# jan-hofmeier/pathnet-gym

Hardware: AMD Instinct MI355X
Metric: env_frames_per_sec_whole_node_pong_pathnet (higher is better)
Workload: dtype fp32x

## Files before the change

csrc/trunk_x3.hip:

```cpp
#include "common.h"
#include <type_traits>

namespace x3 {

#define X3_NCX 3
#define X3_MAXM 16
#define X3_NCT 5
#define X3_RING_FCS 1024
#define X3_C1_FWD_FCS 128
#define X3_W0_SHIFT 8

template <int HIN_, int WIN_, int CIN_, int KH_, int KW_, int S_, bool U8_>
struct CG {
  static constexpr int HIN = HIN_, WIN = WIN_, CIN = CIN_, KH = KH_, KW = KW_, S = S_;
  static constexpr bool U8 = U8_;
  static constexpr int HO = (HIN - KH) / S + 1, WO = (WIN - KW) / S + 1, HOWO = HO * WO;
  static constexpr int K = KH * KW * CIN, KP = (K + 31) / 32 * 32, KC = KP / 8;
  static constexpr int IN_ELEMS = HIN * WIN * CIN;
};
using C1 = CG<160, 120, 4, 8, 8, 4, true>;
using C2 = CG<39, 29, 8, 4, 4, 2, false>;
using C3 = CG<18, 13, 8, 3, 3, 1, false>;

typedef __bf16 b2v __attribute__((ext_vector_type(2)));
// ... 2734 lines not shown

template <int COUT>
__global__ __launch_bounds__(256) void fc_gm_x3(const float* __restrict__ G, const uint16_t* __restrict__ bits,
                                                const int* __restrict__ act_cnt, int layer, int L, int P, int E, int T,
                                                long bits_rows, float g_scale, bf16_t* __restrict__ Gm, long gmlo,
                                                const float* __restrict__ gamax) {
  constexpr int NW = COUT / 16, C8 = COUT / 8;
  const int R = T * E;
  const long idx = (long)blockIdx.x * 256 + threadIdx.x;
  const long row = idx / C8;
  const int c = (int)(idx - row * C8) * 8;
  if (row >= (long)P * R) return;
  const int p = (int)(row / R), r = (int)(row - (long)p * R);
  const int cnt = act_cnt[p * L + layer];
  const long sg = sample_global(p, r, E, P * E, 0);
  const float4 a0 = *reinterpret_cast<const float4*>(G + sg * COUT + c);
  const float4 a1 = *reinterpret_cast<const float4*>(G + sg * COUT + c + 4);
  const float gv[8] = {a0.x * g_scale, a0.y * g_scale, a0.z * g_scale, a0.w * g_scale,
                       a1.x * g_scale, a1.y * g_scale, a1.z * g_scale, a1.w * g_scale};
  const float gs = g16_scale(gamax);
  for (int a = 0; a < cnt; ++a) {
    const uint32_t bw = (uint32_t)bits[((long)a * bits_rows + sg) * NW + (c >> 4)] >> (c & 15);
    float m[8];
#pragma unroll
    for (int j = 0; j < 8; ++j) m[j] = ((bw >> j) & 1u) ? gv[j] : 0.f;
    s8v hi, lo;
    split8hs(m, gs, hi, lo);
    bf16_t* gp = Gm + ((long)a * bits_rows + sg) * COUT + c;
    *reinterpret_cast<s8v*>(gp) = hi;
    *reinterpret_cast<s8v*>(gp + gmlo) = lo;
  }
}

template <int COUT, bool W3 = false, int FOLD = 0>
__global__ __launch_bounds__(512) void fc_dgrad_gemm_x3(const bf16_t* __restrict__ Gm, long gmlo,
                                                        const bf16_t* __restrict__ WcT, long wlo,
                                                        const int* __restrict__ act_idx,
                                                        const int* __restrict__ act_cnt, int layer, int L, int M, int K,
                                                        int KP, int P, int E, int T, long bits_rows,
                                                        float* __restrict__ dX, int nrb, int ncb,
                                                        const float* __restrict__ gamax, float* __restrict__ gamax_out) {
  constexpr int BM = 128, BN = 256, CS = COUT / 32;
  constexpr int NBP = W3 ? 3 : 2;
  __shared__ __attribute__((aligned(16))) bf16_t As[2][2][BM * 32];
  __shared__ __attribute__((aligned(16))) bf16_t Bs[2][NBP][BN * 32];
  const int ntot = P * nrb * ncb, per = (ntot + 7) >> 3, kx = (int)(blockIdx.x >> 3);
  const int bid = (int)(blockIdx.x & 7) * per + kx;
  if (kx >= per || bid >= ntot) return;
  const int p = bid / (nrb * ncb), rem = bid - p * (nrb * ncb);
  const int rbk = rem / ncb, cb = rem - rbk * ncb;
  const int R = T * E, PE = P * E;
  const int cnt = act_cnt[p * L + layer];
  const int tid = threadIdx.x, w = tid >> 6, l = tid & 63;
  const int grp = l >> 4, c16 = l & 15;
  const int wm = w >> 2, wn = w & 3;
  const int row0 = rbk * BM, col0 = cb * BN;
  const int nsteps = cnt * CS;
  f4v acc[4][4], accn[FOLD == 2 ? 4 : 1][FOLD == 2 ? 4 : 1];
#pragma unroll
  for (int i = 0; i < 4; ++i)
#pragma unroll
    for (int jj = 0; jj < 4; ++jj) acc[i][jj] = (f4v){0.f, 0.f, 0.f, 0.f};
  if constexpr (FOLD == 2) {
#pragma unroll
    for (int i = 0; i < 4; ++i)
#pragma unroll
      for (int jj = 0; jj < 4; ++jj) accn[i][jj] = (f4v){0.f, 0.f, 0.f, 0.f};
  }
  if (nsteps > 0) {
    const int sr = tid >> 2, sk = tid & 3;
    const int ra = min(row0 + sr, R - 1);
    const long asg = sample_global(p, ra, E, PE, 0);
    const int kb0 = min(col0 + sr, K - 1), kb1 = min(col0 + 128 + sr, K - 1);
    const int* aidx = act_idx + (p * L + layer) * M;
    const int sdA = mm2_sw(sr, sk) * 8, sdB0 = sdA, sdB1 = mm2_sw(sr + 128, sk) * 8;
    uint4 x0, x1, y0, y1, z0, z1, u0, u1, v0, v1, t0_, t1_, r0, r1, q0, q1;
#define DG_LOAD(S, st)                                                                                      \
    do {                                                                                                    \
      const int a_ = (st) / CS, c_ = ((st) - a_ * CS) * 32 + sk * 8;                                        \
      const bf16_t* ga_ = Gm + ((long)a_ * bits_rows + asg) * COUT + c_;                                    \
      const bf16_t* wb_ = WcT + (long)aidx[a_] * KP * COUT + c_;                                            \
      x##S = *reinterpret_cast<const uint4*>(ga_);                                                          \
      y##S = *reinterpret_cast<const uint4*>(ga_ + gmlo);                                                   \
      z##S = *reinterpret_cast<const uint4*>(wb_ + (long)kb0 * COUT);                                       \
      u##S = *reinterpret_cast<const uint4*>(wb_ + wlo + (long)kb0 * COUT);                                 \
      v##S = *reinterpret_cast<const uint4*>(wb_ + (long)kb1 * COUT);                                       \
      t##S##_ = *reinterpret_cast<const uint4*>(wb_ + wlo + (long)kb1 * COUT);                              \
      if constexpr (W3) {                                                                                   \
        r##S = *reinterpret_cast<const uint4*>(wb_ + 2 * wlo + (long)kb0 * COUT);                           \
        q##S = *reinterpret_cast<const uint4*>(wb_ + 2 * wlo + (long)kb1 * COUT);                           \
      }                                                                                                     \
    } while (0)
#define DG_STORE(S, buf)                                                                                    \
    do {                                                                                                    \
      if (FOLD == 2 && (buf) == 1) {              \
        x##S.x ^= 0x80008000u; x##S.y ^= 0x80008000u; x##S.z ^= 0x80008000u; x##S.w ^= 0x80008000u;         \
        y##S.x ^= 0x80008000u; y##S.y ^= 0x80008000u; y##S.z ^= 0x80008000u; y##S.w ^= 0x80008000u;         \
      }                                                                                                     \
      *reinterpret_cast<uint4*>(&As[buf][0][sdA]) = x##S;                                                   \
      *reinterpret_cast<uint4*>(&As[buf][1][sdA]) = y##S;                                                   \
      *reinterpret_cast<uint4*>(&Bs[buf][0][sdB0]) = z##S;                                                  \
      *reinterpret_cast<uint4*>(&Bs[buf][1][sdB0]) = u##S;                                                  \
      *reinterpret_cast<uint4*>(&Bs[buf][0][sdB1]) = v##S;                                                  \
      *reinterpret_cast<uint4*>(&Bs[buf][1][sdB1]) = t##S##_;                                               \
      if constexpr (W3) {                                                                                   \
        *reinterpret_cast<uint4*>(&Bs[buf][NBP - 1][sdB0]) = r##S;                                          \
        *reinterpret_cast<uint4*>(&Bs[buf][NBP - 1][sdB1]) = q##S;                                          \
      }                                                                                                     \
    } while (0)
    auto compute = [&](int buf) {
      s8v bh[4], bl[4], br[W3 ? 4 : 1];
#pragma unroll
      for (int jj = 0; jj < 4; ++jj) {
        const int o = mm2_sw(wn * 64 + jj * 16 + c16, grp) * 8;
        bh[jj] = *reinterpret_cast<const s8v*>(&Bs[buf][0][o]);
        bl[jj] = *reinterpret_cast<const s8v*>(&Bs[buf][1][o]);
        if constexpr (W3) br[jj] = *reinterpret_cast<const s8v*>(&Bs[buf][NBP - 1][o]);
      }
#pragma unroll
      for (int i = 0; i < 4; ++i) {
        const int o = mm2_sw(wm * 64 + i * 16 + c16, grp) * 8;
        const s8v ah = *reinterpret_cast<const s8v*>(&As[buf][0][o]);
        const s8v al = *reinterpret_cast<const s8v*>(&As[buf][1][o]);
#pragma unroll
        for (int jj = 0; jj < 4; ++jj) {
          if constexpr (FOLD == 2) {
            if (buf == 1) {
// ... 28 lines not shown
    if (s < nsteps) compute(0);
#undef DG_LOAD
#undef DG_STORE
  }
  const float inv = 1.0f / (g16_scale(gamax) * (float)(1 << X3_W0_SHIFT));
  float am = 0.f;
  if constexpr (FOLD == 2) {
#pragma unroll
    for (int i = 0; i < 4; ++i)
#pragma unroll
      for (int jj = 0; jj < 4; ++jj) acc[i][jj] -= accn[i][jj];
  }
#pragma unroll
  for (int i = 0; i < 4; ++i) {
#pragma unroll
    for (int r = 0; r < 4; ++r) {
      const int row = row0 + wm * 64 + i * 16 + 4 * grp + r;
      if (row >= R) continue;
      float* o = dX + sample_global(p, row, E, PE, 0) * (long)K;
#pragma unroll
      for (int jj = 0; jj < 4; ++jj) {
        const int k = col0 + wn * 64 + jj * 16 + c16;
        if (k < K) {
          const float v = acc[i][jj][r] * inv;
          o[k] = v;
          am = fmaxf(am, fabsf(v));
        }
      }
    }
  }
  g16_flush_amax(am, gamax_out);
}

template <int COUT, int KT = 128>
__global__ __launch_bounds__(512) void fc_wgrad_gm_x3(const bf16_t* __restrict__ X, long xlo, int ldx,
                                                      const bf16_t* __restrict__ Gm, long gmlo,
                                                      float* __restrict__ grad, long w_off, long b_off, int chunk,
                                                      const int* __restrict__ inv_path,
                                                      const int* __restrict__ inv_slot,
                                                      const int* __restrict__ inv_cnt, int layer, int M, int Pmax,
                                                      int K, int P, int E, int T, long bits_rows, int nsplit,
                                                      const float* __restrict__ gamax, long long* __restrict__ fx) {
  constexpr int XS = KT + 8;
  constexpr int MI = KT / 64;
  constexpr int XC = KT / 128;
  constexpr int GS = COUT + 8;
  constexpr int NT = COUT / 32;
  __shared__ __attribute__((aligned(16))) bf16_t Xs[2][2][32 * XS];
  __shared__ __attribute__((aligned(16))) bf16_t Gsh[2][2][32 * GS];
  const int kt = (K + KT - 1) / KT;
  const int zt = blockIdx.x / kt, tile_k = blockIdx.x - zt * kt;
  const int j = zt / nsplit, split = zt - j * nsplit;
  const int n_all = inv_cnt[layer * M + j];
  const int u_beg = (int)((long)n_all * split / nsplit), u_end = (int)((long)n_all * (split + 1) / nsplit);
  if (u_beg >= u_end) return;
  const int k0 = tile_k * KT;
  const int tid = threadIdx.x, w = tid >> 6, l = tid & 63;
  const int grp = l >> 4, i16 = l & 15, q = i16 >> 2, pp = i16 & 3;
  const int wk = w >> 1, wn = w & 1;
  const int Rtot = T * E, PE = P * E;
  const int nrb = (Rtot + 31) / 32;
  const int n_it = (u_end - u_beg) * nrb;
  const int* ip = inv_path + (layer * M + j) * Pmax;
  const int* is = inv_slot + (layer * M + j) * Pmax;
  constexpr int GSEG = COUT / 16;
  const int lr = tid >> 4, lxs = (tid & 15) * 8, lgs = (tid & 15) * GSEG;
  s8v xrh[XC], xrl[XC], grh[GSEG / 8], grl[GSEG / 8];
  auto gload = [&](int it) {
    const int ui = it / nrb;
    const int r = (it - ui * nrb) * 32 + lr;
    const int p = ip[u_beg + ui], a = is[u_beg + ui];
    const s8v z = (s8v){0, 0, 0, 0, 0, 0, 0, 0};
#pragma unroll
    for (int c = 0; c < XC; ++c) { xrh[c] = z; xrl[c] = z; }
#pragma unroll
    for (int h = 0; h < GSEG / 8; ++h) { grh[h] = z; grl[h] = z; }
    if (r < Rtot) {
      const long sg = sample_global(p, r, E, PE, 0);
#pragma unroll
      for (int c = 0; c < XC; ++c) {
        if (k0 + lxs + 128 * c < K) {
          xrh[c] = *reinterpret_cast<const s8v*>(X + sg * ldx + k0 + lxs + 128 * c);
          xrl[c] = *reinterpret_cast<const s8v*>(X + xlo + sg * ldx + k0 + lxs + 128 * c);
        }
      }
      const bf16_t* gp = Gm + ((long)a * bits_rows + sg) * COUT + lgs;
#pragma unroll
      for (int h = 0; h < GSEG / 8; ++h) {
        grh[h] = *reinterpret_cast<const s8v*>(gp + 8 * h);
        grl[h] = *reinterpret_cast<const s8v*>(gp + gmlo + 8 * h);
      }
    }
  };
  f4v acc[MI][NT];
#pragma unroll
  for (int i = 0; i < MI; ++i)
#pragma unroll
    for (int jj = 0; jj < NT; ++jj) acc[i][jj] = {0.f, 0.f, 0.f, 0.f};
  float bsum[NT];
#pragma unroll
  for (int jj = 0; jj < NT; ++jj) bsum[jj] = 0.f;
  const bool do_bias = tile_k == 0 && wk == 0;
  gload(0);
  for (int it = 0; it < n_it; ++it) {
    const int buf = it & 1;
#pragma unroll
    for (int c = 0; c < XC; ++c) {
      *reinterpret_cast<s8v*>(Xs[buf][0] + lr * XS + lxs + 128 * c) = xrh[c];
      *reinterpret_cast<s8v*>(Xs[buf][1] + lr * XS + lxs + 128 * c) = xrl[c];
    }
#pragma unroll
    for (int h = 0; h < GSEG / 8; ++h) {
      *reinterpret_cast<s8v*>(Gsh[buf][0] + lr * GS + lgs + 8 * h) = grh[h];
      *reinterpret_cast<s8v*>(Gsh[buf][1] + lr * GS + lgs + 8 * h) = grl[h];
    }
    __syncthreads();
    if (it + 1 < n_it) gload(it + 1);
    s8v afh[MI], afl[MI];
#pragma unroll
    for (int i = 0; i < MI; ++i) {
      const int o0 = (8 * grp + q) * XS + (KT / 4) * wk + 16 * i + 4 * pp;
      const int o1 = (8 * grp + 4 + q) * XS + (KT / 4) * wk + 16 * i + 4 * pp;
      afh[i] = tr8(Xs[buf][0] + o0, Xs[buf][0] + o1);
      afl[i] = tr8(Xs[buf][1] + o0, Xs[buf][1] + o1);
    }
#pragma unroll
    for (int jj = 0; jj < NT; ++jj) {
      const int nb = (COUT / 2) * wn + 16 * jj;
      const int o0 = (8 * grp + q) * GS + nb + 4 * pp, o1 = (8 * grp + 4 + q) * GS + nb + 4 * pp;
      const s8v bh = tr8(Gsh[buf][0] + o0, Gsh[buf][0] + o1);
      const s8v bl = tr8(Gsh[buf][1] + o0, Gsh[buf][1] + o1);
#pragma unroll
      for (int i = 0; i < MI; ++i) acc[i][jj] = mma3h(afh[i], afl[i], bh, bl, acc[i][jj]);
      if (do_bias) {
#pragma unroll
        for (int e = 0; e < 8; ++e) bsum[jj] += h2f((uint16_t)bh[e]) + h2f((uint16_t)bl[e]);
      }
    }
  }
  const long base = w_off + (long)j * chunk;
  const float ginv = 1.0f / g16_scale(gamax);
#pragma unroll
  for (int i = 0; i < MI; ++i)
#pragma unroll
    for (int jj = 0; jj < NT; ++jj)
// ... 244 lines not shown
  return Hin == G::HIN && Win == G::WIN && Cin == G::CIN && KH == G::KH && KW == G::KW && S == G::S &&
         (u8 != 0) == G::U8;
}

static int X3_WGRAD_PF = 3;
static int X3_C1_WG_NCX = 2;
static int X3_FC_KS = 1;
static int X3_FC_MMV = 3;
static int X3_FC_FWD_WPE = 0;
static int X3_C1_F16B = 1;
static int X3_C1_SB1 = 0;
static int X3_C1_EMAJ = 1;
static int X3_C1_BAL = 1;
static int X3_DG_W3 = 0;
static int X3_DG_FOLD = 2;
static int X3_WG_TARGET = 1536;
static int X3_WG_AUTO = 1;
static int X3_WG2_TARGET = 512;
static int X3_DG3_TARGET = 512;
static int X3_FC_RT1 = 2;
static int X3_C1F_TARGET = 512;
static int X3_C1F_MINB = 2;
static int X3_C23_TARGET = 512;
static int X3_C23_MINS = 1;
static int X3_WG3_TARGET = 256;
static int X3_FCW_TARGET = 1024;
static int X3_PRESPLIT = 1;
static int X3_DG_BAL = 1;
static int X3_DG_V0 = 0;
static int X3_DG_GSPLIT = X3_DG_SPLIT;
static int X3_DG_TARGET = 512;
static int X3_FC_KS_PARTS = 0;
static int X3_FC_DG_GEMM = 1;

template <auto KERN, int CAP>
static size_t lds_cap_pad() {
  static const size_t pad = [] {
    hipFuncAttributes a;
    if (hipFuncGetAttributes(&a, reinterpret_cast<const void*>(KERN)) != hipSuccess) return (size_t)0;
    const long need = 160L * 1024 / (CAP + 1) + 1;
    return need > (long)a.sharedSizeBytes ? (size_t)(need - (long)a.sharedSizeBytes) : (size_t)0;
  }();
  return pad;
}

long long* g_fx_accum = nullptr;

extern "C" {

int x3_set_fx(void* fx) {
  g_fx_accum = reinterpret_cast<long long*>(fx);
  return 0;
}

int x3_fx_flush(void* fx, float* grad, long n0, long n1, hipStream_t st) {
  if (!fx || !grad || n0 < 0 || n1 < n0) return -22;
  if (n1 == n0) return 0;
  long blocks = (n1 - n0 + 255) / 256;
  if (blocks > 2048) blocks = 2048;
  fx_flush_kernel<<<(unsigned)blocks, 256, 0, st>>>(reinterpret_cast<long long*>(fx), grad, n0, n1);
  return (int)hipGetLastError();
}

void fast_conv_set_x3_c1_wg_ncx(int v) { X3_C1_WG_NCX = v == 2 ? 2 : 3; }
void fast_conv_set_x3_fc_mmv(int v) { X3_FC_MMV = v; }
void fast_conv_set_x3_fc_fwd_wpe(int v) { X3_FC_FWD_WPE = v == 2 || v == 4 ? v : 0; }
void fast_conv_set_x3_fc_dg_gemm(int v) { X3_FC_DG_GEMM = v; }
void fast_conv_set_x3_dg_w3(int v) { X3_DG_W3 = v; }
void fast_conv_set_x3_dg_fold(int v) { X3_DG_FOLD = v; }
void fast_conv_set_x3_dg_v0(int v) { X3_DG_V0 = v; }
void fast_conv_set_x3_dg_bal(int v) { X3_DG_BAL = v; }
void fast_conv_set_x3_dg_gsplit(int v) { X3_DG_GSPLIT = v == 1 ? 1 : X3_DG_SPLIT; }
void fast_conv_set_x3_c1_bal(int v) { X3_C1_BAL = v; }
void fast_conv_set_x3_c1_emaj(int v) { X3_C1_EMAJ = v; }
void fast_conv_set_x3_c1_sb1(int v) { X3_C1_SB1 = v; }
void fast_conv_set_x3_c1_f16b(int v) { X3_C1_F16B = v; }
void fast_conv_set_x3_fc_ks(int ks) { X3_FC_KS = ks; }
void fast_conv_set_x3_wgrad_pf(int pf) { X3_WGRAD_PF = pf; }
void fast_conv_set_x3_presplit(int v) { X3_PRESPLIT = v ? 1 : 0; }
void fast_conv_set_x3_fc_rt1(int v) { X3_FC_RT1 = v; }
void fast_conv_set_x3_c1f_target(int v) { X3_C1F_TARGET = v < 1 ? 1 : v; }
void fast_conv_set_x3_c1f_minb(int v) { X3_C1F_MINB = v < 1 ? 1 : v; }
void fast_conv_set_x3_c23_target(int v) { X3_C23_TARGET = v < 1 ? 1 : v; }
void fast_conv_set_x3_c23_mins(int v) { X3_C23_MINS = v < 1 ? 1 : v; }
void fast_conv_set_x3_wg3_target(int v) { X3_WG3_TARGET = v < 1 ? 1 : v; }
void fast_conv_set_x3_fcw_target(int v) { X3_FCW_TARGET = v < 1 ? 1 : v; }
void fast_conv_set_x3_wg2_target(int v) { X3_WG2_TARGET = v < 0 ? 0 : v; }
void fast_conv_set_x3_dg3_target(int v) { X3_DG3_TARGET = v < 0 ? 0 : v; }
void fast_conv_set_x3_wg_auto(int v) { X3_WG_AUTO = v; }
void fast_conv_set_x3_wg_target(int v) { X3_WG_TARGET = v < 0 ? 0 : v; }
void fast_conv_set_x3_dg_target(int v) { X3_DG_TARGET = v < 0 ? 0 : v; }
void fast_conv_set_x3_fc_ks_parts(int v) { X3_FC_KS_PARTS = (v == 2 || v == 3 || v == 4 || v == 8) ? v : 0; }

int x3_conv_fwd(const void* X, long xlo, int u8in, void* Y, long ylo, void* bits, const void* Wc, long wlo,
                const float* flat, long bias_off, int chunk, const int* ai, const int* ac, int layer, int L, int M,
                int Hin, int Win, int Cin, int KH, int KW, int S, int P, int E, int T, int t0, long br, float is,
                float os, hipStream_t st) {
  if (chunk <= 0 || L <= 0 || M <= 0 || Hin <= 0 || Win <= 0 || Cin <= 0 || KH <= 0 || KW <= 0 || S <= 0 || P <= 0 ||
      E <= 0 || T <= 0 || br <= 0 || u8in < 0 || bias_off < 0 || layer < 0 || t0 < 0 || xlo < 0 || ylo <= 0 ||
      wlo <= 0) return -22;
// ... 365 lines not shown
                                          wlo, flat, bias_off, chunk, inv_path, inv_slot, inv_cnt, layer, M, KP, P, E, \
                                          T, t0, br, isc)
    if (KP == 256) FMM(8); else FMM(0);
#undef FMM
  }
  int rc = (int)hipGetLastError();
  if (rc) return -rc;
  const long thr = (long)P * R * 32;
  const unsigned g2 = (unsigned)((thr + 255) / 256);
  if (ylo == 0)
    fc_slot_sum_x3<true><<<g2, 256, 0, st>>>(Ys, ac, layer, L, P, E, T, t0, Y, 0, os);
  else
    fc_slot_sum_x3<false><<<g2, 256, 0, st>>>(Ys, ac, layer, L, P, E, T, t0, Y, ylo, os);
  rc = (int)hipGetLastError();
  return rc ? -rc : 1;
}

int x3_fc_dgrad(const float* G, const void* bits, const void* WcT, long wlo, const int* ai, const int* ac, int layer,
                int L, int M, int K, int KP, int Cout, int P, int E, int T, long br, float gs, float* dX, void* Gm,
                long gmlo, const float* gamax, float* gamax_out, hipStream_t st) {
  if (L <= 0 || M <= 0 || K <= 0 || KP <= 0 || Cout <= 0 || P <= 0 || E <= 0 || T <= 0 || br <= 0 || layer < 0 ||
      wlo <= 0 || gmlo < 0 || (Gm && gmlo <= 0) || !gamax) return -22;
  if (M > X3_MAXM || Cout != 256) return 0;
  if (X3_FC_DG_GEMM && Gm != nullptr) {
    const int R = T * E;
    const long thr = (long)P * R * (256 / 8);
    fc_gm_x3<256><<<(unsigned)((thr + 255) / 256), 256, 0, st>>>(G, (const uint16_t*)bits, ac, layer, L, P, E, T, br,
                                                                  gs, (bf16_t*)Gm, gmlo, gamax);
    int rc = (int)hipGetLastError();
    if (rc) return -rc;
    const int nrb = (R + 127) / 128, ncb = (K + 255) / 256;
    const unsigned nwg = (unsigned)((P * nrb * ncb + 7) / 8 * 8);
#define DGG(W3_, FOLD_)                                                                                           \
    fc_dgrad_gemm_x3<256, W3_, FOLD_><<<nwg, 512, 0, st>>>((const bf16_t*)Gm, gmlo, (const bf16_t*)WcT, wlo, ai, ac, \
                                                           layer, L, M, K, KP, P, E, T, br, dX, nrb, ncb, gamax,     \
                                                           gamax_out)
    if (X3_DG_FOLD == 2) DGG(false, 2);
    else if (X3_DG_W3 && X3_DG_FOLD) DGG(true, 1);
    else if (X3_DG_W3) DGG(true, 0);
    else if (X3_DG_FOLD) DGG(false, 1);
    else DGG(false, 0);
#undef DGG
    rc = (int)hipGetLastError();
    return rc ? -rc : 1;
  }
  const int nchunks = (K + 127) / 128;
  const int split = nchunks >= 8 ? 2 : 1;
  const int per = (nchunks + split - 1) / split;
  const int nrowb = (int)(((long)T * E + 63) / 64);
  const int nwg = (nrowb * P * split + 7) / 8 * 8;
  fc_dgrad_x3<256><<<nwg, 512, 0, st>>>(G, (const uint16_t*)bits, (const bf16_t*)WcT, wlo, ai, ac, layer, L, M, K, KP,
                                        P, E, T, br, gs, dX, per, nrowb, split, (bf16_t*)Gm, gmlo, gamax, gamax_out);
  const int rc = (int)hipGetLastError();
  return rc ? -rc : 1;
}

int x3_fc_wgrad_gm(const void* X, long xlo, int ldx, const void* Gm, long gmlo, float* grad, long w_off, long b_off,
                   int chunk, const int* inv_path, const int* inv_slot, const int* inv_cnt, int layer, int M, int Pmax,
                   int K, int Cout, int P, int E, int T, long br, int nsplit, const float* gamax, hipStream_t st) {
  if (ldx <= 0 || chunk <= 0 || M <= 0 || Pmax <= 0 || K <= 0 || Cout <= 0 || P <= 0 || E <= 0 || T <= 0 || br <= 0 ||
      nsplit <= 0 || w_off < 0 || b_off < 0 || layer < 0 || xlo <= 0 || gmlo <= 0 || !gamax) return -22;
  if (Cout != 256 || ldx % 8 != 0 || K % 8 != 0) return 0;
  if (K > 256) {
    const int kt = (K + 255) / 256;
    fc_wgrad_gm_x3<256, 256><<<kt * M * nsplit, 512, 0, st>>>((const bf16_t*)X, xlo, ldx, (const bf16_t*)Gm, gmlo,
                                                              grad, w_off, b_off, chunk, inv_path, inv_slot, inv_cnt,
                                                              layer, M, Pmax, K, P, E, T, br, nsplit, gamax,
                                                              g_fx_accum);
  } else {
    const int kt = (K + 127) / 128;
    fc_wgrad_gm_x3<256><<<kt * M * nsplit, 512, 0, st>>>((const bf16_t*)X, xlo, ldx, (const bf16_t*)Gm, gmlo, grad,
                                                         w_off, b_off, chunk, inv_path, inv_slot, inv_cnt, layer, M,
                                                         Pmax, K, P, E, T, br, nsplit, gamax, g_fx_accum);
  }
  const int rc = (int)hipGetLastError();
  return rc ? -rc : 1;
}

int x3_fc_wgrad(const void* X, long xlo, int ldx, const float* G, const void* bits, float* grad, long w_off,
                long b_off, int chunk, const int* inv_path, const int* inv_slot, const int* inv_cnt, int layer, int M,
                int Pmax, int K, int Cout, int P, int E, int T, long br, float gs, const float* gamax, hipStream_t st) {
  if (ldx <= 0 || chunk <= 0 || M <= 0 || Pmax <= 0 || K <= 0 || Cout <= 0 || P <= 0 || E <= 0 || T <= 0 || br <= 0 ||
      w_off < 0 || b_off < 0 || layer < 0 || xlo <= 0 || !gamax) return -22;
  if (Cout % 16 != 0 || ldx % 8 != 0) return 0;
  const int tiles = ((K + 63) / 64) * ((Cout + 63) / 64) * M;
  int nsplit = (X3_FCW_TARGET + tiles - 1) / tiles;
  nsplit = nsplit < 1 ? 1 : (nsplit > Pmax ? Pmax : nsplit);
  fc_wgrad_x3<<<dim3((K + 63) / 64, (Cout + 63) / 64, M * nsplit), 256, 0, st>>>(
      (const bf16_t*)X, xlo, ldx, G, (const uint16_t*)bits, grad, w_off, b_off, chunk, inv_path, inv_slot, inv_cnt,
      layer, M, Pmax, K, Cout, P, E, T, br, gs, nsplit, gamax, g_fx_accum);
  const int rc = (int)hipGetLastError();
  return rc ? -rc : 1;
}

__global__ __launch_bounds__(256) void x3_amax_kernel(const float* __restrict__ g, long n, float* __restrict__ amax) {
  float m = 0.f;
  for (long i = ((long)blockIdx.x * 256 + threadIdx.x) * 4; i < n; i += (long)gridDim.x * 256 * 4) {
    if (i + 3 < n) {
      const float4 v = *reinterpret_cast<const float4*>(g + i);
      m = fmaxf(m, fmaxf(fmaxf(fabsf(v.x), fabsf(v.y)), fmaxf(fabsf(v.z), fabsf(v.w))));
    } else {
      for (long j = i; j < n; ++j) m = fmaxf(m, fabsf(g[j]));
    }
  }
  g16_flush_amax_wg(m, amax);
}
__global__ void x3_amax_reset_kernel(float* __restrict__ amax, int n) {
// ... 55 lines not shown
```

pathnet_gym_amd/ops/_lib.py:

```python
from __future__ import annotations

import ctypes
import os
from ctypes import c_float, c_int, c_long, c_uint, c_void_p, c_size_t

import torch

_HERE = os.path.dirname(os.path.abspath(__file__))
LIB_PATH = os.path.join(os.path.dirname(_HERE), "_hip", "libpathnet_hip.so")

P = c_void_p
_SIGS = {
    "launch_conv_fwd": [P, c_int, P, P, P, P, c_long, c_int, P, P, c_int, c_int, c_int, c_int, c_int, c_int, c_int,
                        c_int, c_int, c_int, c_int, c_int, c_int, c_int, c_int, c_int, c_int, c_long, c_float,
                        c_float, P],
    "launch_fc_fwd": [P, c_int, P, P, P, P, c_long, c_int, P, P, c_int, c_int, c_int, c_int, c_int, c_int, c_int,
                      c_int, c_int, c_int, c_long, c_float, P],
    "launch_conv_wgrad": [P, c_int, P, P, P, c_long, c_long, c_int, P, P, c_int, c_int, c_int, c_int, c_int, c_int,
                          c_int, c_int, c_int, c_int, c_int, c_int, c_int, c_int, c_int, c_int, c_long, c_int,
                          c_float, c_float, P],
    "launch_conv_dgrad": [P, P, P, c_long, c_int, P, P, c_int, c_int, c_int, c_int, c_int, c_int, c_int, c_int,
                          c_int, c_int, c_int, c_int, c_int, c_int, c_long, c_float, P, P],
    "launch_fc_dgrad": [P, P, P, P, P, c_int, c_int, c_int, c_int, c_int, c_int, c_int, c_int, c_int, c_long, c_float,
                        P, P, P],
# ... 104 lines not shown
    "launch_refresh_weights_f32": [P, c_long, c_int, c_int, c_int, c_int, c_int, P, P, P],
    "launch_heads_bwd_det": [P, c_int, c_int, P, P, c_int, c_int, P, c_long, c_long, c_long, c_long, P, P, P, P],
    "heads_bwd_part_numel": [c_int, c_int, c_int],
    "heads_bwd_split_numel": [c_int, c_int, c_int],
    "launch_heads_bwd_split": [P, c_int, c_int, P, P, c_int, c_int, P, c_long, c_long, c_long, c_long, P, P, P, P],
    "fast_conv_dgrad_bf16": [P, c_int, P, P, c_long, c_int, P, P, c_int, c_int, c_int, c_int, c_int, c_int, c_int,
                             c_int, c_int, c_int, c_int, c_int, c_long, c_float, P, c_int, P],
    "fast_conv_wgrad_bf16g": [P, c_int, P, P, P, c_long, c_long, c_int, P, P, c_int, c_int, c_int, c_int, c_int, c_int,
                              c_int, c_int, c_int, c_int, c_int, c_int, c_long, c_float, c_float, P],
    "x3_conv_fwd": [P, c_long, c_int, P, c_long, P, P, c_long, P, c_long, c_int, P, P] + [c_int] * 13
                   + [c_long, c_float, c_float, P],
    "x3_conv_wgrad": [P, c_long, c_int, P, P, P, c_long, c_long, c_int, P, P] + [c_int] * 12
                     + [c_long, c_float, c_float, P, P],
    "x3_conv1_ring_fwd": [P, P, P, c_long, P, P, c_long, P, c_long, c_int, P, P] + [c_int] * 8
                         + [c_long, c_float, c_float, P],
    "x3_conv23_fwd": [P, c_long, P, c_long, P, c_long, P, c_long, c_long, c_int, P, c_long, P, c_long, P, c_long,
                      c_long, c_int, P, P, P] + [c_int] * 7 + [c_float, c_float, P],
    "x3_conv1_ring_wgrad": [P, P, P, P, P, c_long, c_long, c_int, P, P] + [c_int] * 7 + [c_long, c_float, c_float, P,
                                                                                         P],
    "x3_conv_dgrad": [P, P, P, c_long, c_int, P, P] + [c_int] * 12 + [c_long, c_float, P, P, P, P],
    "x3_fc_fwd": [P, c_long, c_int, P, c_long, P, P, c_long, P, c_long, c_int, P, P] + [c_int] * 10
                 + [c_long, c_float, P],
    "x3_fc_heads_fwd": [P, c_long, c_int, P, P, P, c_long, P, c_long, c_int, P, P] + [c_int] * 9
                       + [c_long, c_float, c_long, c_long, c_long, c_long, c_int, P, P, P, c_uint, P, c_int, c_int,
                          c_int, c_uint, P],
    "x3_fc_fwd_mm": [P, c_long, c_int, P, c_long, P, P, c_long, P, c_long, c_int, P, P, P, P, P, P] + [c_int] * 10
                    + [c_long, c_float, P],
    "x3_fc_dgrad": [P, P, P, c_long, P, P] + [c_int] * 9 + [c_long, c_float, P, P, c_long, P, P, P],
    "x3_amax": [P, c_long, P, P],
    "x3_amax_reset": [P, c_int, P],
    "x3_fc_wgrad_gm": [P, c_long, c_int, P, c_long, P, c_long, c_long, c_int, P, P, P] + [c_int] * 8
                      + [c_long, c_int, P, P],
    "x3_fc_wgrad": [P, c_long, c_int, P, P, P, c_long, c_long, c_int, P, P, P] + [c_int] * 8 + [c_long, c_float, P, P],
    "x3_refresh_weights": [P, c_long, c_int, c_int, c_int, c_int, c_int, P, P, c_int, P, P],
    "x3_status_fold": [P, P, P],
    "x3_set_fx": [P],
    "x3_fx_flush": [P, P, c_long, c_long, P],
    "fast_conv_set_x3_fc_mmv": [c_int],
    "fast_conv_set_x3_fc_fwd_wpe": [c_int],
    "fast_conv_set_x3_fc_dg_gemm": [c_int],
    "fast_conv_set_x3_dg_w3": [c_int],
    "fast_conv_set_x3_c1_f16b": [c_int],
    "fast_conv_set_x3_dg_fold": [c_int],
    "heads_set_s16": [c_int],
    "heads_set_bwd_rows": [c_int],
    "fast_conv_set_x3_fc_ks": [c_int],
    "fast_conv_set_x3_wgrad_pf": [c_int],
    "fast_conv_set_x3_c1_wg_ncx": [c_int],
    "fast_conv_set_x3_wg_target": [c_int],
    "fast_conv_set_x3_wg_auto": [c_int],
    "fast_conv_set_x3_wg2_target": [c_int],
    "fast_conv_set_x3_wg3_target": [c_int],
    "fast_conv_set_x3_c1f_target": [c_int],
    "fast_conv_set_x3_fc_rt1": [c_int],
    "fast_conv_set_x3_c1f_minb": [c_int],
    "fast_conv_set_x3_c23_target": [c_int],
    "fast_conv_set_x3_c23_mins": [c_int],
    "fast_conv_set_x3_fcw_target": [c_int],
    "fast_conv_set_x3_dg3_target": [c_int],
    "fast_conv_set_x3_c1_sb1": [c_int],
    "fast_conv_set_x3_presplit": [c_int],
    "fast_conv_set_x3_dg_target": [c_int],
    "fast_conv_set_x3_fc_ks_parts": [c_int],
    "conv_fwd_smem": [c_int, c_int],
    "conv_wgrad_smem": [c_int],
}
# ... 60 lines not shown
```

pathnet_gym_amd/ops/pathnet_ops.py:

```python
from __future__ import annotations

import ctypes
import os
from dataclasses import dataclass
from typing import List, Optional

import numpy as np
import torch

from . import _lib


def round_up(x, m):
    return (x + m - 1) // m * m


def x2_alloc(shape, device) -> torch.Tensor:
    return torch.zeros((2,) + tuple(shape), dtype=torch.float16, device=device)[0]


def x2_lo(t: torch.Tensor) -> int:
    nb = t.untyped_storage().nbytes()
    if t.dtype != torch.float16 or nb % 4 != 0 or t.storage_offset() + t.numel() > nb // 4:
        raise ValueError("not plane 0 of a fp16-pair allocation (x2_alloc)")
# ... 653 lines not shown
        return self._ys

    def _gamax(self, l: int):
        return None if l < 0 else self.gamax.data_ptr() + 4 * l

    def _layer_bwd_x3(self, l, X, G, bits, grad_flat, dX, P, E, T, bits_rows, g_scale, st, part=None):
        g = self.geoms[l]
        m = self.model
        flat = m.store.flat
        do_w, do_d = part in (None, "w"), part in (None, "d")
        _lib.check(G, torch.float32, name="G")
        if dX is not None:
            _lib.check(dX, torch.float32, name="dX")
        if l == self.L - 1 and do_d:
            _lib.call("x3_amax_reset", self.gamax.data_ptr(), self.L, st)
            _lib.call("x3_amax", G.data_ptr(), G.numel(), self._gamax(l), st)
        ga, ga_out = self._gamax(l), self._gamax(l - 1)
        xb, xblo = self._x3_bf16(X)
        if g.kind == "conv":
            ok = True
            if do_w:
                ok = _lib.call_fast("x3_conv_wgrad", xb, xblo, int(g.u8in), G.data_ptr(),
                                    bits.data_ptr(), grad_flat.data_ptr(), g.w_off, g.b_off, g.chunk,
                                    m.act_idx.data_ptr(), m.act_cnt.data_ptr(), l, self.L, self.M, g.Hin, g.Win, g.Cin,
                                    g.KH, g.KW, g.S, P, E, T, bits_rows, g.in_scale, g_scale, ga, st)
            if ok and dX is not None and do_d:
                ok = _lib.call_fast("x3_conv_dgrad", G.data_ptr(), bits.data_ptr(), flat.data_ptr(), g.w_off, g.chunk,
                                    m.act_idx.data_ptr(), m.act_cnt.data_ptr(), l, self.L, self.M, g.Hin, g.Win, g.Cin,
                                    g.KH, g.KW, g.S, P, E, T, bits_rows, g_scale, dX.data_ptr(), ga, ga_out, st)
            if not ok:
                raise RuntimeError(f"fp32x: conv layer {l} backward has no split-bf16 kernel")
            return
        use_gm_wgrad = dX is not None and g.Cout == 256 and g.K >= self.fc_wgrad_gm_min_k and self.fc_wgrad_gm
        gm = self._gm_buffer_x3(bits_rows) if (dX is not None and g.Cout == 256) else None
        gmlo = gm.numel() // 2 if gm is not None else 0
        ok = True
        if dX is not None and do_d:
            ok = _lib.call_fast("x3_fc_dgrad", G.data_ptr(), bits.data_ptr(), self.WcT[l].data_ptr(),
                                self.WcT[l][0].numel(), m.act_idx.data_ptr(), m.act_cnt.data_ptr(), l, self.L, self.M,
                                g.K, g.KP, g.Cout, P, E, T, bits_rows, g_scale, dX.data_ptr(), _lib.ptr(gm), gmlo, ga,
                                ga_out, st)
        if not do_w:
            pass
        elif ok and use_gm_wgrad:
            tiles = ((g.K + 127) // 128) * self.M
            wgs = self.fc_wgrad_gm_wgs if m.P > 16 else self.fc_wgrad_gm_wgs_small
            nsplit = max(1, min(m.P, -(-wgs // tiles)))
            ok = _lib.call_fast("x3_fc_wgrad_gm", xb, xblo, g.ldx, gm.data_ptr(), gmlo,
                                grad_flat.data_ptr(), g.w_off, g.b_off, g.chunk, self.inv_path.data_ptr(),
                                self.inv_slot.data_ptr(), self.inv_cnt.data_ptr(), l, self.M, m.P, g.K, g.Cout, P, E, T,
                                bits_rows, nsplit, ga, st)
        elif ok:
            ok = _lib.call_fast("x3_fc_wgrad", xb, xblo, g.ldx, G.data_ptr(), bits.data_ptr(),
                                grad_flat.data_ptr(), g.w_off, g.b_off, g.chunk, self.inv_path.data_ptr(),
                                self.inv_slot.data_ptr(), self.inv_cnt.data_ptr(), l, self.M, m.P, g.K, g.Cout, P, E, T,
                                bits_rows, g_scale, ga, st)
        if not ok:
            raise RuntimeError(f"fp32x: fc layer {l} backward has no split-bf16 kernel")

    def _gm_buffer_x3(self, bits_rows: int) -> torch.Tensor:
        n = 2 * self.M * bits_rows * 256
        buf = getattr(self, "_gm", None)
        if buf is None or buf.numel() != n:
            buf = torch.empty(n, dtype=torch.bfloat16, device=self.model.store.flat.device)
            self._gm = buf
        return buf

    def _layer_fwd_f32(self, l, xp, yp, bp, aip, acp, P, E, T, t0, bits_rows, out_scale, st):
        g = self.geoms[l]
        flat = self.model.store.flat
        if g.kind == "conv":
            if (E * g.HWo) % 16 != 0:
                raise ValueError(f"layer {l}: envs_per_path*Ho*Wo must be a multiple of 16")
            _lib.call("launch_conv_fwd_f32", xp, int(g.u8in), yp, bp,
                      self.Wc[l].data_ptr(), flat.data_ptr(), g.b_off, g.chunk, aip,
                      acp, l, self.L, self.M, g.Hin, g.Win, g.Cin, g.KH, g.KW, g.S, g.Ho, g.Wo,
                      g.K, g.KP, P, E, T, t0, bits_rows, g.in_scale, out_scale, st)
        else:
            _lib.call("launch_fc_fwd_f32", xp, g.ldx, yp, bp, self.Wc[l].data_ptr(),
                      flat.data_ptr(), g.b_off, g.chunk, aip, acp, l, self.L,
                      self.M, g.K, g.KP, g.Cout, P, E, T, t0, bits_rows, out_scale, st)

    def wgrad_chunks(self, l: int, P: int, E: int, T: int) -> int:
        g = self.geoms[l]
        rows = T * E * g.HWo
        want = max(1, min(-(-rows // 32), -(-1024 // P)))
        rpc = round_up(-(-rows // want), 32)
        return -(-rows // rpc)

    def _part_buffer(self, numel: int) -> torch.Tensor:
        if self._part is None or self._part.numel() < numel:
            self._part = torch.empty(numel, dtype=torch.float32, device=self.model.store.flat.device)
        return self._part

    def _layer_bwd_bf16_grads(self, l, X, G, bits, grad_flat, dX, P, E, T, bits_rows, g_scale, st):
        g = self.geoms[l]
        m = self.model
        flat = m.store.flat
        if g.kind != "conv":
            raise RuntimeError(f"layer {l}: bf16 activation gradients are for the conv layers")
# ... 244 lines not shown
```

Baseline: 3.949 million.

## Split FC gradient once and apply activation mask inside dgrad/wgrad loads

Instead of materialising a per-module masked split-bf16 gradient buffer (M copies of the gradient), the FC backward now splits the gradient once into a single hi/lo buffer and applies the per-module activation bitmask when tiles are loaded into LDS in both the dgrad GEMM and the wgrad kernel. This is meant to cut global memory writes and reads proportional to the number of modules. In exchange it adds bitmask loads and masking ALU work in the inner load path. It also adds an optional split-major block ordering for wgrad, which is off by default.

New measurement: 3.932 million. About the same (-0.4%).

```diff
diff --git a/csrc/trunk_x3.hip b/csrc/trunk_x3.hip
--- a/csrc/trunk_x3.hip
+++ b/csrc/trunk_x3.hip
@@ -2790,8 +2790,32 @@
   }
 }
 
-template <int COUT, bool W3 = false, int FOLD = 0>
+template <int COUT>
+__global__ __launch_bounds__(256) void fc_gsplit_x3(const float* __restrict__ G, int P, int E, int T, float g_scale,
+                                                    bf16_t* __restrict__ Gs, long gslo,
+                                                    const float* __restrict__ gamax) {
+  constexpr int C8 = COUT / 8;
+  const int R = T * E;
+  const long idx = (long)blockIdx.x * 256 + threadIdx.x;
+  const long row = idx / C8;
+  const int c = (int)(idx - row * C8) * 8;
+  if (row >= (long)P * R) return;
+  const int p = (int)(row / R), r = (int)(row - (long)p * R);
+  const long sg = sample_global(p, r, E, P * E, 0);
+  const float4 a0 = *reinterpret_cast<const float4*>(G + sg * COUT + c);
+  const float4 a1 = *reinterpret_cast<const float4*>(G + sg * COUT + c + 4);
+  const float gv[8] = {a0.x * g_scale, a0.y * g_scale, a0.z * g_scale, a0.w * g_scale,
+                       a1.x * g_scale, a1.y * g_scale, a1.z * g_scale, a1.w * g_scale};
+  s8v hi, lo;
+  split8hs(gv, g16_scale(gamax), hi, lo);
+  bf16_t* gp = Gs + sg * COUT + c;
+  *reinterpret_cast<s8v*>(gp) = hi;
+  *reinterpret_cast<s8v*>(gp + gslo) = lo;
+}
+
+template <int COUT, bool W3 = false, int FOLD = 0, bool GS = false>
 __global__ __launch_bounds__(512) void fc_dgrad_gemm_x3(const bf16_t* __restrict__ Gm, long gmlo,
+                                                        const uint8_t* __restrict__ bits,
                                                         const bf16_t* __restrict__ WcT, long wlo,
                                                         const int* __restrict__ act_idx,
                                                         const int* __restrict__ act_cnt, int layer, int L, int M, int K,
@@ -2833,10 +2857,12 @@
     const int* aidx = act_idx + (p * L + layer) * M;
     const int sdA = mm2_sw(sr, sk) * 8, sdB0 = sdA, sdB1 = mm2_sw(sr + 128, sk) * 8;
     uint4 x0, x1, y0, y1, z0, z1, u0, u1, v0, v1, t0_, t1_, r0, r1, q0, q1;
+    uint32_t m0 = 0, m1 = 0;
 #define DG_LOAD(S, st)                                                                                      \
     do {                                                                                                    \
       const int a_ = (st) / CS, c_ = ((st) - a_ * CS) * 32 + sk * 8;                                        \
-      const bf16_t* ga_ = Gm + ((long)a_ * bits_rows + asg) * COUT + c_;                                    \
+      const bf16_t* ga_ = Gm + (GS ? asg : (long)a_ * bits_rows + asg) * COUT + c_;                         \
+      if constexpr (GS) m##S = bits[((long)a_ * bits_rows + asg) * (COUT / 8) + (c_ >> 3)];                 \
       const bf16_t* wb_ = WcT + (long)aidx[a_] * KP * COUT + c_;                                            \
       x##S = *reinterpret_cast<const uint4*>(ga_);                                                          \
       y##S = *reinterpret_cast<const uint4*>(ga_ + gmlo);                                                   \
@@ -2851,6 +2877,12 @@
     } while (0)
 #define DG_STORE(S, buf)                                                                                    \
     do {                                                                                                    \
+      if constexpr (GS) {                                                                                   \
+        s8v mh_, ml_;                                                                                       \
+        mask_pair8(__builtin_bit_cast(s8v, x##S), __builtin_bit_cast(s8v, y##S), m##S, mh_, ml_);           \
+        x##S = __builtin_bit_cast(uint4, mh_);                                                              \
+        y##S = __builtin_bit_cast(uint4, ml_);                                                              \
+      }                                                                                                     \
       if (FOLD == 2 && (buf) == 1) {              \
         x##S.x ^= 0x80008000u; x##S.y ^= 0x80008000u; x##S.z ^= 0x80008000u; x##S.w ^= 0x80008000u;         \
         y##S.x ^= 0x80008000u; y##S.y ^= 0x80008000u; y##S.z ^= 0x80008000u; y##S.w ^= 0x80008000u;         \
@@ -2945,15 +2977,17 @@
   g16_flush_amax(am, gamax_out);
 }
 
-template <int COUT, int KT = 128>
+template <int COUT, int KT = 128, bool GSPLIT = false>
 __global__ __launch_bounds__(512) void fc_wgrad_gm_x3(const bf16_t* __restrict__ X, long xlo, int ldx,
                                                       const bf16_t* __restrict__ Gm, long gmlo,
+                                                      const uint16_t* __restrict__ bits,
                                                       float* __restrict__ grad, long w_off, long b_off, int chunk,
                                                       const int* __restrict__ inv_path,
                                                       const int* __restrict__ inv_slot,
                                                       const int* __restrict__ inv_cnt, int layer, int M, int Pmax,
                                                       int K, int P, int E, int T, long bits_rows, int nsplit,
-                                                      const float* __restrict__ gamax, long long* __restrict__ fx) {
+                                                      int smajor, const float* __restrict__ gamax,
+                                                      long long* __restrict__ fx) {
   constexpr int XS = KT + 8;
   constexpr int MI = KT / 64;
   constexpr int XC = KT / 128;
@@ -2963,7 +2997,7 @@
   __shared__ __attribute__((aligned(16))) bf16_t Gsh[2][2][32 * GS];
   const int kt = (K + KT - 1) / KT;
   const int zt = blockIdx.x / kt, tile_k = blockIdx.x - zt * kt;
-  const int j = zt / nsplit, split = zt - j * nsplit;
+  const int j = smajor ? zt % M : zt / nsplit, split = smajor ? zt / M : zt - j * nsplit;
   const int n_all = inv_cnt[layer * M + j];
   const int u_beg = (int)((long)n_all * split / nsplit), u_end = (int)((long)n_all * (split + 1) / nsplit);
   if (u_beg >= u_end) return;
@@ -2979,6 +3013,7 @@
   constexpr int GSEG = COUT / 16;
   const int lr = tid >> 4, lxs = (tid & 15) * 8, lgs = (tid & 15) * GSEG;
   s8v xrh[XC], xrl[XC], grh[GSEG / 8], grl[GSEG / 8];
+  uint32_t gbw = 0;
   auto gload = [&](int it) {
     const int ui = it / nrb;
     const int r = (it - ui * nrb) * 32 + lr;
@@ -2988,6 +3023,7 @@
     for (int c = 0; c < XC; ++c) { xrh[c] = z; xrl[c] = z; }
 #pragma unroll
     for (int h = 0; h < GSEG / 8; ++h) { grh[h] = z; grl[h] = z; }
+    if constexpr (GSPLIT) gbw = 0;
     if (r < Rtot) {
       const long sg = sample_global(p, r, E, PE, 0);
 #pragma unroll
@@ -2997,7 +3033,8 @@
           xrl[c] = *reinterpret_cast<const s8v*>(X + xlo + sg * ldx + k0 + lxs + 128 * c);
         }
       }
-      const bf16_t* gp = Gm + ((long)a * bits_rows + sg) * COUT + lgs;
+      const bf16_t* gp = Gm + (GSPLIT ? sg : (long)a * bits_rows + sg) * COUT + lgs;
+      if constexpr (GSPLIT) gbw = bits[((long)a * bits_rows + sg) * (COUT / 16) + (lgs >> 4)];
 #pragma unroll
       for (int h = 0; h < GSEG / 8; ++h) {
         grh[h] = *reinterpret_cast<const s8v*>(gp + 8 * h);
@@ -3024,6 +3061,7 @@
     }
 #pragma unroll
     for (int h = 0; h < GSEG / 8; ++h) {
+      if constexpr (GSPLIT) mask_pair8(grh[h], grl[h], gbw >> (8 * h), grh[h], grl[h]);
       *reinterpret_cast<s8v*>(Gsh[buf][0] + lr * GS + lgs + 8 * h) = grh[h];
       *reinterpret_cast<s8v*>(Gsh[buf][1] + lr * GS + lgs + 8 * h) = grl[h];
     }
@@ -3334,6 +3372,8 @@
 static int X3_DG_TARGET = 512;
 static int X3_FC_KS_PARTS = 0;
 static int X3_FC_DG_GEMM = 1;
+static int X3_FC_GMASK = 1;
+static int X3_FCW_ORDER = 0;
 
 template <auto KERN, int CAP>
 static size_t lds_cap_pad() {
@@ -3368,6 +3408,8 @@
 void fast_conv_set_x3_fc_mmv(int v) { X3_FC_MMV = v; }
 void fast_conv_set_x3_fc_fwd_wpe(int v) { X3_FC_FWD_WPE = v == 2 || v == 4 ? v : 0; }
 void fast_conv_set_x3_fc_dg_gemm(int v) { X3_FC_DG_GEMM = v; }
+void fast_conv_set_x3_fc_gmask(int v) { X3_FC_GMASK = v ? 1 : 0; }
+void fast_conv_set_x3_fcw_order(int v) { X3_FCW_ORDER = v ? 1 : 0; }
 void fast_conv_set_x3_dg_w3(int v) { X3_DG_W3 = v; }
 void fast_conv_set_x3_dg_fold(int v) { X3_DG_FOLD = v; }
 void fast_conv_set_x3_dg_v0(int v) { X3_DG_V0 = v; }
@@ -3799,9 +3841,9 @@
     const int nrb = (R + 127) / 128, ncb = (K + 255) / 256;
     const unsigned nwg = (unsigned)((P * nrb * ncb + 7) / 8 * 8);
 #define DGG(W3_, FOLD_)                                                                                           \
-    fc_dgrad_gemm_x3<256, W3_, FOLD_><<<nwg, 512, 0, st>>>((const bf16_t*)Gm, gmlo, (const bf16_t*)WcT, wlo, ai, ac, \
-                                                           layer, L, M, K, KP, P, E, T, br, dX, nrb, ncb, gamax,     \
-                                                           gamax_out)
+    fc_dgrad_gemm_x3<256, W3_, FOLD_><<<nwg, 512, 0, st>>>((const bf16_t*)Gm, gmlo, nullptr, (const bf16_t*)WcT, wlo, \
+                                                           ai, ac, layer, L, M, K, KP, P, E, T, br, dX, nrb, ncb,     \
+                                                           gamax, gamax_out)
     if (X3_DG_FOLD == 2) DGG(false, 2);
     else if (X3_DG_W3 && X3_DG_FOLD) DGG(true, 1);
     else if (X3_DG_W3) DGG(true, 0);
@@ -3831,15 +3873,71 @@
   if (K > 256) {
     const int kt = (K + 255) / 256;
     fc_wgrad_gm_x3<256, 256><<<kt * M * nsplit, 512, 0, st>>>((const bf16_t*)X, xlo, ldx, (const bf16_t*)Gm, gmlo,
-                                                              grad, w_off, b_off, chunk, inv_path, inv_slot, inv_cnt,
-                                                              layer, M, Pmax, K, P, E, T, br, nsplit, gamax,
-                                                              g_fx_accum);
+                                                              nullptr, grad, w_off, b_off, chunk, inv_path, inv_slot,
+                                                              inv_cnt, layer, M, Pmax, K, P, E, T, br, nsplit,
+                                                              X3_FCW_ORDER, gamax, g_fx_accum);
   } else {
     const int kt = (K + 127) / 128;
-    fc_wgrad_gm_x3<256><<<kt * M * nsplit, 512, 0, st>>>((const bf16_t*)X, xlo, ldx, (const bf16_t*)Gm, gmlo, grad,
-                                                         w_off, b_off, chunk, inv_path, inv_slot, inv_cnt, layer, M,
-                                                         Pmax, K, P, E, T, br, nsplit, gamax, g_fx_accum);
-  }
+    fc_wgrad_gm_x3<256><<<kt * M * nsplit, 512, 0, st>>>((const bf16_t*)X, xlo, ldx, (const bf16_t*)Gm, gmlo, nullptr,
+                                                         grad, w_off, b_off, chunk, inv_path, inv_slot, inv_cnt, layer,
+                                                         M, Pmax, K, P, E, T, br, nsplit, X3_FCW_ORDER, gamax,
+                                                         g_fx_accum);
+  }
+  const int rc = (int)hipGetLastError();
+  return rc ? -rc : 1;
+}
+
+int x3_fc_gmask_active() { return X3_FC_GMASK && X3_FC_DG_GEMM; }
+
+int x3_fc_gsplit(const float* G, int Cout, int P, int E, int T, float gs, void* Gs, long gslo, const float* gamax,
+                 hipStream_t st) {
+  if (!G || !Gs || Cout <= 0 || P <= 0 || E <= 0 || T <= 0 || gslo <= 0 || !gamax) return -22;
+  if (Cout != 256) return 0;
+  const long thr = (long)P * T * E * (256 / 8);
+  if ((thr + 255) / 256 > 0x7FFFFFFFL || gslo < (long)P * T * E * 256) return -22;
+  fc_gsplit_x3<256><<<(unsigned)((thr + 255) / 256), 256, 0, st>>>(G, P, E, T, gs, (bf16_t*)Gs, gslo, gamax);
+  const int rc = (int)hipGetLastError();
+  return rc ? -rc : 1;
+}
+
+int x3_fc_dgrad_masked(const void* Gs, long gslo, const void* bits, const void* WcT, long wlo, const int* ai,
+                       const int* ac, int layer, int L, int M, int K, int KP, int Cout, int P, int E, int T, long br,
+                       float* dX, const float* gamax, float* gamax_out, hipStream_t st) {
+  if (L <= 0 || M <= 0 || K <= 0 || KP <= 0 || Cout <= 0 || P <= 0 || E <= 0 || T <= 0 || br <= 0 || layer < 0 ||
+      wlo <= 0 || gslo <= 0 || !Gs || !bits || !gamax) return -22;
+  if (M > X3_MAXM || Cout != 256) return 0;
+  const long R = (long)T * E, nrb = (R + 127) / 128, ncb = (K + 255) / 256;
+  if (br < (long)P * R || gslo < (long)P * R * 256 || (long)P * nrb * ncb + 7 > 0x7FFFFFFFL) return -22;
+  const unsigned nwg = (unsigned)(((long)P * nrb * ncb + 7) / 8 * 8);
+#define DGG(W3_, FOLD_)                                                                                           \
+  fc_dgrad_gemm_x3<256, W3_, FOLD_, true><<<nwg, 512, 0, st>>>((const bf16_t*)Gs, gslo, (const uint8_t*)bits,     \
+                                                               (const bf16_t*)WcT, wlo, ai, ac, layer, L, M, K, KP, \
+                                                               P, E, T, br, dX, (int)nrb, (int)ncb, gamax, gamax_out)
+  if (X3_DG_FOLD == 2) DGG(false, 2);
+  else if (X3_DG_W3 && X3_DG_FOLD) DGG(true, 1);
+  else if (X3_DG_W3) DGG(true, 0);
+  else if (X3_DG_FOLD) DGG(false, 1);
+  else DGG(false, 0);
+#undef DGG
+  const int rc = (int)hipGetLastError();
+  return rc ? -rc : 1;
+}
+
+int x3_fc_wgrad_gs(const void* X, long xlo, int ldx, const void* Gs, long gslo, const void* bits, float* grad,
+                   long w_off, long b_off, int chunk, const int* inv_path, const int* inv_slot, const int* inv_cnt,
+                   int layer, int M, int Pmax, int K, int Cout, int P, int E, int T, long br, int nsplit,
+                   const float* gamax, hipStream_t st) {
+  if (ldx <= 0 || chunk <= 0 || M <= 0 || Pmax <= 0 || K <= 0 || Cout <= 0 || P <= 0 || E <= 0 || T <= 0 || br <= 0 ||
+      nsplit <= 0 || w_off < 0 || b_off < 0 || layer < 0 || xlo <= 0 || gslo <= 0 || !Gs || !bits || !gamax) return -22;
+  if (Cout != 256 || ldx % 8 != 0 || K % 8 != 0) return 0;
+  const long kt = K > 256 ? (K + 255) / 256 : (K + 127) / 128;
+  if (gslo < (long)P * T * E * 256 || kt * M * nsplit > 0x7FFFFFFFL) return -22;
+#define WGS(KT_)                                                                                                  \
+  fc_wgrad_gm_x3<256, KT_, true><<<(unsigned)(kt * M * nsplit), 512, 0, st>>>(                                    \
+      (const bf16_t*)X, xlo, ldx, (const bf16_t*)Gs, gslo, (const uint16_t*)bits, grad, w_off, b_off, chunk, inv_path, \
+      inv_slot, inv_cnt, layer, M, Pmax, K, P, E, T, br, nsplit, X3_FCW_ORDER, gamax, g_fx_accum)
+  if (K > 256) WGS(256); else WGS(128);
+#undef WGS
   const int rc = (int)hipGetLastError();
   return rc ? -rc : 1;
 }
diff --git a/pathnet_gym_amd/ops/_lib.py b/pathnet_gym_amd/ops/_lib.py
--- a/pathnet_gym_amd/ops/_lib.py
+++ b/pathnet_gym_amd/ops/_lib.py
@@ -160,6 +160,13 @@
     "x3_fc_wgrad_gm": [P, c_long, c_int, P, c_long, P, c_long, c_long, c_int, P, P, P] + [c_int] * 8
                       + [c_long, c_int, P, P],
     "x3_fc_wgrad": [P, c_long, c_int, P, P, P, c_long, c_long, c_int, P, P, P] + [c_int] * 8 + [c_long, c_float, P, P],
+    "x3_fc_gmask_active": [],
+    "x3_fc_gsplit": [P, c_int, c_int, c_int, c_int, c_float, P, c_long, P, P],
+    "x3_fc_dgrad_masked": [P, c_long, P, P, c_long, P, P] + [c_int] * 9 + [c_long, P, P, P, P],
+    "x3_fc_wgrad_gs": [P, c_long, c_int, P, c_long, P, P, c_long, c_long, c_int, P, P, P] + [c_int] * 8
+                      + [c_long, c_int, P, P],
+    "fast_conv_set_x3_fc_gmask": [c_int],
+    "fast_conv_set_x3_fcw_order": [c_int],
     "x3_refresh_weights": [P, c_long, c_int, c_int, c_int, c_int, c_int, P, P, c_int, P, P],
     "x3_status_fold": [P, P, P],
     "x3_set_fx": [P],
diff --git a/pathnet_gym_amd/ops/pathnet_ops.py b/pathnet_gym_amd/ops/pathnet_ops.py
--- a/pathnet_gym_amd/ops/pathnet_ops.py
+++ b/pathnet_gym_amd/ops/pathnet_ops.py
@@ -709,6 +709,32 @@
                 raise RuntimeError(f"fp32x: conv layer {l} backward has no split-bf16 kernel")
             return
         use_gm_wgrad = dX is not None and g.Cout == 256 and g.K >= self.fc_wgrad_gm_min_k and self.fc_wgrad_gm
+        if dX is not None and g.Cout == 256 and _lib.lib().x3_fc_gmask_active():
+            gs = self._gs_buffer_x3(bits_rows)
+            gslo = gs.numel() // 2
+            ok = True
+            if do_d:
+                ok = _lib.call_fast("x3_fc_gsplit", G.data_ptr(), g.Cout, P, E, T, g_scale, gs.data_ptr(), gslo, ga, st)
+                ok = ok and _lib.call_fast("x3_fc_dgrad_masked", gs.data_ptr(), gslo, bits.data_ptr(),
+                                           self.WcT[l].data_ptr(), self.WcT[l][0].numel(), m.act_idx.data_ptr(),
+                                           m.act_cnt.data_ptr(), l, self.L, self.M, g.K, g.KP, g.Cout, P, E, T,
+                                           bits_rows, dX.data_ptr(), ga, ga_out, st)
+            if ok and do_w and use_gm_wgrad:
+                tiles = ((g.K + 127) // 128) * self.M
+                wgs = self.fc_wgrad_gm_wgs if m.P > 16 else self.fc_wgrad_gm_wgs_small
+                nsplit = max(1, min(m.P, -(-wgs // tiles)))
+                ok = _lib.call_fast("x3_fc_wgrad_gs", xb, xblo, g.ldx, gs.data_ptr(), gslo, bits.data_ptr(),
+                                    grad_flat.data_ptr(), g.w_off, g.b_off, g.chunk, self.inv_path.data_ptr(),
+                                    self.inv_slot.data_ptr(), self.inv_cnt.data_ptr(), l, self.M, m.P, g.K, g.Cout, P,
+                                    E, T, bits_rows, nsplit, ga, st)
+            elif ok and do_w:
+                ok = _lib.call_fast("x3_fc_wgrad", xb, xblo, g.ldx, G.data_ptr(), bits.data_ptr(),
+                                    grad_flat.data_ptr(), g.w_off, g.b_off, g.chunk, self.inv_path.data_ptr(),
+                                    self.inv_slot.data_ptr(), self.inv_cnt.data_ptr(), l, self.M, m.P, g.K, g.Cout, P,
+                                    E, T, bits_rows, g_scale, ga, st)
+            if not ok:
+                raise RuntimeError(f"fp32x: fc layer {l} backward has no split-bf16 kernel")
+            return
         gm = self._gm_buffer_x3(bits_rows) if (dX is not None and g.Cout == 256) else None
         gmlo = gm.numel() // 2 if gm is not None else 0
         ok = True
@@ -743,6 +769,14 @@
             self._gm = buf
         return buf
 
+    def _gs_buffer_x3(self, bits_rows: int) -> torch.Tensor:
+        n = 2 * bits_rows * 256
+        buf = getattr(self, "_gs", None)
+        if buf is None or buf.numel() != n:
+            buf = torch.empty(n, dtype=torch.bfloat16, device=self.model.store.flat.device)
+            self._gs = buf
+        return buf
+
     def _layer_fwd_f32(self, l, xp, yp, bp, aip, acp, P, E, T, t0, bits_rows, out_scale, st):
         g = self.geoms[l]
         flat = self.model.store.flat
```
